# wulibingbinglin/COMET-Pose-Estimation

Measured on AMD Instinct MI355X. Metric: sequences/sec (BxT frames) COMET fwd+bwd, T=16 512^2, higher is better.
Workload: dtype bf16; 1 GPU; train_e2epose2.py fwd+bwd (COMET tracker+DINOv2+head, loss, backward, grad all-reduce, clip 1.0, AdamW) -- BASELINE configs[2]; global_batch=8, seq_len=16, image=512, tracks=512, parallelism=dp1

## Files before the change

### comet-pose-estimation_amd/comet_amd/_lib.py

```python
import ctypes
import os

_HERE = os.path.dirname(os.path.abspath(__file__))
_DEFAULT_LIB = "libcomet_hip_debug.so" if os.environ.get("COMET_DEBUG") == "1" else "libcomet_hip.so"
LIB_PATH = os.environ.get("COMET_HIP_LIB", os.path.join(os.path.dirname(_HERE), _DEFAULT_LIB))

F32 = 0
BF16 = 1
ACT_NONE, ACT_GELU, ACT_RELU, ACT_SIGMOID = 0, 1, 2, 3
SQ_NORM_PARTIALS = 1024

c_i64 = ctypes.c_int64
c_i32 = ctypes.c_int32
c_vp = ctypes.c_void_p


class GemmArgs(ctypes.Structure):
    _fields_ = [
        ("dtype_ab", c_i32), ("dtype_c", c_i32), ("layout_a", c_i32), ("layout_b", c_i32),
        ("m", c_i64), ("n", c_i64), ("k", c_i64), ("batch", c_i64 * 2),
        ("a", c_vp), ("lda", c_i64), ("stride_a", c_i64 * 2),
        ("b", c_vp), ("ldb", c_i64), ("stride_b", c_i64 * 2),
        ("c", c_vp), ("ldc", c_i64), ("stride_c", c_i64 * 2),
        ("bias", c_vp), ("bias_mode", c_i32), ("stride_bias", c_i64 * 2),
# ... 22 lines not shown
        ("bias", c_vp),
        ("y", c_vp), ("ldy", c_i64),
        ("resid", c_vp), ("ldr", c_i64), ("beta", ctypes.c_float),
        ("act", c_i32),
    ]


class AttnArgs(ctypes.Structure):
    _fields_ = [
        ("dtype", c_i32), ("head_dim", c_i32),
        ("batch", c_i64), ("heads", c_i64), ("lq", c_i64), ("lk", c_i64),
        ("q", c_vp), ("sq_b", c_i64), ("sq_h", c_i64), ("sq_l", c_i64),
        ("k", c_vp), ("sk_b", c_i64), ("sk_h", c_i64), ("sk_l", c_i64),
        ("v", c_vp), ("sv_b", c_i64), ("sv_h", c_i64), ("sv_l", c_i64),
        ("o", c_vp), ("so_b", c_i64), ("so_h", c_i64), ("so_l", c_i64),
        ("lse", c_vp), ("scale", ctypes.c_float),
        ("batch_inner", c_i64), ("sq_i", c_i64), ("sk_i", c_i64), ("sv_i", c_i64), ("so_i", c_i64),
    ]


class AttnBwdArgs(ctypes.Structure):
    _fields_ = [
        ("dtype", c_i32), ("head_dim", c_i32),
        ("batch", c_i64), ("heads", c_i64), ("lq", c_i64), ("lk", c_i64),
        ("q", c_vp), ("sq_b", c_i64), ("sq_h", c_i64), ("sq_l", c_i64),
        ("k", c_vp), ("sk_b", c_i64), ("sk_h", c_i64), ("sk_l", c_i64),
        ("v", c_vp), ("sv_b", c_i64), ("sv_h", c_i64), ("sv_l", c_i64),
        ("o", c_vp), ("so_b", c_i64), ("so_h", c_i64), ("so_l", c_i64),
        ("dout", c_vp), ("sd_b", c_i64), ("sd_h", c_i64), ("sd_l", c_i64),
        ("dq", c_vp), ("sdq_b", c_i64), ("sdq_h", c_i64), ("sdq_l", c_i64),
        ("dk", c_vp), ("sdk_b", c_i64), ("sdk_h", c_i64), ("sdk_l", c_i64),
        ("dv", c_vp), ("sdv_b", c_i64), ("sdv_h", c_i64), ("sdv_l", c_i64),
        ("lse", c_vp), ("delta", c_vp), ("scale", ctypes.c_float),
    ]


class RingTensor(ctypes.Structure):
    _fields_ = [("src", c_vp), ("dst", c_vp), ("slot_bytes", c_i64)]


RING_MAX_TENSORS = 4
FUSE_ROW = 20
CARRY_MAX_TRACKS, CARRY_MAX_CANDIDATES, CARRY_MAX_CELLS = 4096, 65536, 8192
LM_ROW = 12
PNP_MAX_ITERS = 16

_F = ctypes.c_float
_INT = ctypes.c_int
SIGNATURES = {
    "comet_count_nonfinite": (_INT, [_INT, c_vp, c_i64, c_vp, c_vp]),
    "comet_debug_flags": (_INT, [_INT]),
    "comet_lds_probe": (_INT, [_INT, _INT, _INT, c_vp, c_vp]),
    "comet_shfl_probe": (_INT, [_INT, _INT, _INT, c_vp, c_vp]),
    "comet_version": (_INT, []),
    "comet_last_error": (ctypes.c_char_p, []),
    "comet_gemm": (_INT, [ctypes.POINTER(GemmArgs), c_vp]),
    "comet_gemm_workspace": (_INT, [ctypes.POINTER(GemmArgs), ctypes.POINTER(c_i64)]),
    "comet_gemm_plan": (_INT, [ctypes.POINTER(GemmArgs), ctypes.POINTER(c_i64), ctypes.POINTER(ctypes.c_int32)]),
    "comet_gemm_rowln_ok": (_INT, [ctypes.POINTER(GemmArgs)]),
    "comet_gemm_rowln_workspace": (_INT, [ctypes.POINTER(GemmArgs), ctypes.POINTER(ctypes.c_int64)]),
    "comet_gemm_rowln": (_INT, [ctypes.POINTER(GemmArgs), ctypes.POINTER(RowLNArgs), c_vp]),
    "comet_gemm_dact_ok": (_INT, [ctypes.POINTER(GemmArgs), _INT, c_vp, c_i64]),
    "comet_gemm_dact": (_INT, [ctypes.POINTER(GemmArgs), _INT, c_vp, c_i64, c_vp, c_vp]),
    "comet_conv2d_nhwc": (_INT, [ctypes.POINTER(ConvArgs), c_vp]),
    "comet_conv_plan": (_INT, [ctypes.POINTER(ConvArgs), ctypes.POINTER(ctypes.c_int32)]),
    "comet_layernorm_fwd": (_INT, [_INT, _INT, c_vp, c_vp, c_vp, c_vp, c_vp, c_vp, c_vp, c_i64, c_i64, c_i64, c_i64,
                                   c_i64, _F, _INT, c_vp]),
    "comet_layernorm_bwd": (_INT, [_INT, _INT, c_vp, c_vp, c_vp, c_vp, c_vp, c_vp, _INT, c_vp, c_vp, c_vp, c_i64, c_i64,
                                   _INT, c_vp]),
    "comet_layernorm_bwd_res": (_INT, [_INT, _INT, c_vp, c_vp, c_vp, c_vp, c_vp, c_vp, c_vp, c_vp, c_vp, c_i64, c_i64,
                                       c_vp]),
    "comet_attention_bwd": (_INT, [ctypes.POINTER(AttnBwdArgs), c_vp]),
    "comet_attention_fwd": (_INT, [ctypes.POINTER(AttnArgs), c_vp]),
    "comet_attn_probs": (_INT, [_INT, c_vp, c_vp, c_vp, c_i64, c_i64, c_i64, c_i64, _F, c_vp]),
    "comet_attn_delta": (_INT, [_INT, c_vp, c_vp, c_vp, c_i64, c_i64, c_i64, c_i64, c_i64, c_i64, c_i64, c_i64, c_i64, c_i64, c_vp]),
    "comet_attn_dsoftmax": (_INT, [_INT, c_vp, c_vp, c_vp, c_vp, c_i64, c_i64, c_i64, _F, c_vp]),
    "comet_cast": (_INT, [_INT, _INT, c_vp, c_vp, c_i64, c_vp]),
    "comet_cast_multi_f32_bf16": (_INT, [c_vp, c_vp, c_vp, _INT, c_vp]),
    "comet_act_bwd": (_INT, [_INT, _INT, _INT, c_vp, c_vp, c_vp, _INT, c_i64, c_vp]),
    "comet_axpby": (_INT, [c_vp, c_vp, _F, _F, c_i64, c_vp]),
    "comet_act_bwd_colsum": (_INT, [_INT, _INT, c_vp, _INT, c_vp, _INT, c_vp, c_vp, c_i64, c_i64, _INT, c_vp]),
    "comet_colsum": (_INT, [_INT, c_vp, c_vp, c_i64, c_i64, c_i64, _INT, c_vp]),
    "comet_sq_norm_multi": (_INT, [c_vp, c_vp, _INT, c_vp, c_vp, c_vp]),
    "comet_adamw_multi": (_INT, [c_vp, c_vp, c_vp, c_vp, c_vp, _INT, _F, _F, _F, _F, _F, _INT, c_vp, _F, c_vp]),
    "comet_im2col_nhwc": (_INT, [_INT, _INT, c_vp, c_vp, c_i64, c_i64, c_i64, c_i64, _INT, _INT, _INT, _INT, c_i64, c_i64, c_i64, c_vp]),
    "comet_instnorm_workspace": (_INT, [c_i64, c_i64, c_i64, ctypes.POINTER(c_i64)]),
    "comet_instnorm_nhwc": (_INT, [_INT, c_vp, c_vp, c_vp, c_i64, c_i64, c_i64, _F, _INT, _INT, c_vp, c_i64, c_vp]),
    "comet_resize_bilinear": (_INT, [_INT, _INT, _INT, c_vp, c_vp, c_i64, c_i64, c_i64, c_i64, c_i64, c_i64, _INT, c_vp]),
    "comet_resize_bilinear_pool_nhwc": (_INT, [_INT, _INT, c_vp, c_vp, c_vp, c_i64, c_i64, c_i64, c_i64, c_i64, c_i64, c_vp]),
    "comet_conv1x1_resize_pool_nhwc": (_INT, [c_vp, c_vp, c_i64, c_i64, c_vp, c_i64, c_i64, c_vp, c_vp, c_vp, c_vp, c_vp,
                                               c_i64, c_i64, c_i64, c_i64, c_i64, c_i64, c_vp]),
    "comet_shallow_front_nhwc": (_INT, [_INT, c_vp, c_vp, c_vp, c_vp, c_vp, c_vp, c_i64, c_i64, c_i64, _F, c_vp]),
    "comet_resize_bilinear_nhwc_into": (_INT, [_INT, _INT, c_vp, c_vp, c_i64, c_i64, c_i64, c_i64, c_i64, c_i64, c_i64,
                                               _INT, c_vp]),
    "comet_act_fwd": (_INT, [_INT, _INT, _INT, c_vp, c_vp, c_i64, c_vp]),
    "comet_binary": (_INT, [_INT, _INT, c_vp, c_vp, c_vp, c_i64, c_vp]),
    "comet_add_rows": (_INT, [_INT, _INT, c_vp, c_vp, c_vp, c_i64, c_i64, c_i64, c_i64, c_i64, c_vp]),
    "comet_rowscale_fwd": (_INT, [_INT, c_vp, c_vp, c_vp, c_i64, c_i64, c_vp]),
    "comet_rowscale_bwd": (_INT, [_INT, c_vp, c_vp, c_vp, c_vp, c_vp, c_i64, c_i64, c_vp]),
    "comet_sincos_table": (_INT, [c_vp, c_vp, c_i64, _INT, c_i64, c_i64, c_vp]),
    "comet_harmonic_fwd": (_INT, [c_vp, c_vp, c_vp, c_vp, c_i64, _INT, _INT, _INT, c_vp]),
    "comet_pose_pair_errors": (_INT, [c_vp, c_vp, c_i64, c_i64, c_vp, c_vp, c_vp]),
    "comet_pose_frame_errors": (_INT, [c_vp, c_i64, c_vp, c_i64, c_i64, c_vp, c_vp, c_vp, c_vp]),
    "comet_harmonic_bwd": (_INT, [c_vp, c_vp, c_vp, c_vp, c_vp, c_vp, c_i64, _INT, _INT, _INT, c_vp]),
# ... 77 lines not shown
```

### comet-pose-estimation_amd/comet_amd/functional.py

```python
import contextlib

import os

import torch

from . import _lib as L
from . import ops


class _State:
    dtype = torch.bfloat16


_state = _State()


def compute_dtype():
    return _state.dtype


@contextlib.contextmanager
def precision(dtype):
    old = _state.dtype
    _state.dtype = dtype
# ... 561 lines not shown
        dw = torch.zeros(C, device=x.device) if ctx.needs_input_grad[1] else None
        db = torch.zeros(C, device=x.device) if ctx.needs_input_grad[2] else None
        dx = ops.layernorm_bwd(x, dpre, mean, rstd, w, dw, db) if (ctx.needs_input_grad[0] or dw is not None or db is not None) else None
        return dx, dw, db, None


def layer_norm_relu(x, w, b, eps=1e-5):
    if _needs_grad(x, w, b):
        return _LayerNormReLU.apply(x, w, b, eps)
    return ops.layernorm(x, w, b, eps=eps, out_dtype=torch.float32, relu=True)


class _RowScale(torch.autograd.Function):

    @staticmethod
    def forward(ctx, x, w):
        ctx.save_for_backward(x, w)
        return ops.rowscale(x, w)

    @staticmethod
    def backward(ctx, dy):
        x, w = ctx.saved_tensors
        dx, dw = ops.rowscale_bwd(x, w, dy, ctx.needs_input_grad[0], ctx.needs_input_grad[1])
        return dx, dw


def rowscale(x, w):
    w = w.reshape(x.shape[:-1])
    if _needs_grad(x, w):
        return _RowScale.apply(x, w)
    return ops.rowscale(x, w)


class _Add(torch.autograd.Function):
    @staticmethod
    def forward(ctx, a, b):
        return ops.add(a, b)

    @staticmethod
    def backward(ctx, g):
        return g, g


def add(a, b):
    if _needs_grad(a, b):
        return _Add.apply(a, b)
    return ops.add(a, b)


class _AddRows(torch.autograd.Function):
    @staticmethod
    def forward(ctx, x, table, period):
        return ops.add_rows(x, table, period, out_dtype=torch.float32)

    @staticmethod
    def backward(ctx, g):
        return g, None, None


def add_rows(x, table, period):
    if _needs_grad(x):
        return _AddRows.apply(x, table, period)
    return ops.add_rows(x, table, period, out_dtype=torch.float32)


class _GAPR(torch.autograd.Function):
# ... 89 lines not shown
```

### comet-pose-estimation_amd/comet_amd/models/camera_predictor10.py

```python
import math

import torch
import torch.nn as nn

from .. import _lib as L
from .. import functional as F
from .. import ops
from .dinov2 import dinov2_vitb14_reg
from .modules import AttnBlock, CrossAttnBlock, Mlp
from .utils import INTRINSICS, PredCameras

_RESNET_MEAN = [0.485, 0.456, 0.406]
_RESNET_STD = [0.229, 0.224, 0.225]


class FeatureFusion(nn.Module):

    def __init__(self, rgb_dim, fmap_dim, fusion_type="adaptive"):
        super().__init__()
        self.fusion_type = fusion_type
        self.fmap_proj = nn.Sequential(nn.Linear(fmap_dim, rgb_dim), nn.LayerNorm(rgb_dim), nn.ReLU())
        self.fusion_layer = nn.Linear(rgb_dim * 2, rgb_dim)
        self.out_norm = nn.LayerNorm(rgb_dim)

# ... 146 lines not shown
        blk, cblk = self.self_att[-1], self.cross_att[-1]
        a = blk.attn
        x = tok.reshape(B * S, P, C)
        xn, xc = F.layer_norm_dual(x, eps=1e-6)
        idx = self._query_rows(B, S, P, x.device)
        qin = F.gather_rows(xc.reshape(B * S * P, C), idx)
        rin = F.gather_rows(xn.reshape(B * S * P, C), idx)
        q, kv = F.linear_pair(qin, xc, a.in_proj_weight, a.in_proj_bias, C)
        o0 = F.attention(q[:B * P].reshape(B, P, C), kv.reshape(B, S, P, 2 * C)[:, 0], blk.heads, C)
        o1 = F.attention(q[B * P:].reshape(B * S, 1, C), kv, blk.heads, C)
        o = torch.cat([o0.reshape(B * P, C), o1.reshape(B * S, C)])
        y = F.linear(o, a.out_proj.weight, a.out_proj.bias, resid=rin, out_dtype=torch.float32)
        yr, yn = F.res_layer_norm(y, eps=1e-6)
        y = blk.mlp(yn, resid=yr)
        f0 = y[:B * P].reshape(B, P, C)
        rows = y[B * P:].reshape(B, S, C)[:, 1:].contiguous()
        r = cblk(rows, f0)
        return torch.cat([f0[:, 0:1], r], dim=1)

    def forward(self, reshaped_image, preliminary_cameras=None, iters=4, batch_size=None, rgb_feat_init=None,
                gt_cameras=None, fmaps=None, pred_trajectories=None, track_confidence=None, debug=False,
                tokens=None):
        if rgb_feat_init is None:
            rgb_feat, B, S, C = self.get_2D_image_features(reshaped_image, batch_size, tokens=tokens)
        else:
            rgb_feat = rgb_feat_init
            B, S, C = rgb_feat.shape
        if pred_trajectories is not None and self.USE_TP and self.TP_RESIDUAL:
            traj = self.traj_encoder(pred_trajectories)
            N = traj.shape[2]
            ca = self.confidence_attention
            w = F.linear(track_confidence.unsqueeze(-1), ca[0].weight, ca[0].bias, act=L.ACT_RELU)
            w = F.linear(w, ca[2].weight, ca[2].bias, act=L.ACT_SIGMOID, out_dtype=torch.float32)
            ctx = F.rowscale(traj, w).reshape(B * S, N, C)
            r = rgb_feat.reshape(B * S, 1, C)
            for blk in self.cross_attn_block:
                r = blk(r, ctx)
            rgb_feat = F.add(rgb_feat, r.reshape(B, S, C))
        if self.USE_TIME:
            rgb_feat = F.add_rows(rgb_feat, self._table("1d", S, C, rgb_feat.device), S)
            with F.precision(torch.float32):
                for blk in self.trunk:
                    rgb_feat = blk(rgb_feat)
        if self.SINGLE_HEAD:
            return self._single_head(rgb_feat, gt_cameras, B, S)
        gt_enc = None
        if gt_cameras is not None:
            gt_enc = ops.pose_encode(gt_cameras.R.float(), gt_cameras.T_uvz.float(), gt_cameras.focal_length.float(),
                                     _ratio(gt_cameras), B, S)
        rot = self.pose_branch(rgb_feat)
        uv = F.linear(rgb_feat, self.fc_translation2d.weight, self.fc_translation2d.bias, out_dtype=torch.float32)
        dd = F.linear(rgb_feat, self.fc_depth.weight, self.fc_depth.bias, out_dtype=torch.float32)
        enc, losses = F.gapr(rot, uv, dd, gt_enc, B, S, self._cfg_get("weight_trans", 1), self._cfg_get("weight_rot", 2))
        pred_cameras = None
        if gt_cameras is not None:
            intr = INTRINSICS[_dataset(self.cfg)]
            R, T = ops.pose_decode(enc, gt_cameras.R.float(), gt_cameras.T_uvz.float(), _ratio(gt_cameras), intr, B, S)
            pred_cameras = PredCameras(R=R, T=T, focal_length=torch.zeros(B * S, 0, device=R.device))
        out = {"pred_pose_enc": enc, "gt_pose_enc": gt_enc, "pred_cameras": pred_cameras}
        if gt_enc is not None:
            out.update(loss=losses[0], loss_trans=losses[1], loss_rot=losses[2])
        else:
            out.update(loss=0, loss_trans=0, loss_rot=0)
        return out

    def _single_head(self, rgb_feat, gt_cameras, B, S):
        pred = self.pose_branch(rgb_feat)
        gt8 = None
        if gt_cameras is not None:
            gt8 = ops.pose_encode3(gt_cameras.R.float(), gt_cameras.T.float(), B, S)
# ... 24 lines not shown
```

### comet-pose-estimation_amd/comet_amd/models/modules.py

```python

import torch
import torch.nn as nn

from .. import _lib as L
from .. import functional as F
from .. import ops


class Mlp(nn.Module):
    def __init__(self, in_features, hidden_features=None, out_features=None, act_layer=nn.GELU,
                 norm_layer=None, bias=True, drop=0.0, use_conv=False):
        super().__init__()
        out_features = out_features or in_features
        hidden_features = hidden_features or in_features
        self.fc1 = nn.Linear(in_features, hidden_features, bias=bias)
        self.act = act_layer()
        self.drop1 = nn.Dropout(drop)
        self.fc2 = nn.Linear(hidden_features, out_features, bias=bias)
        self.drop2 = nn.Dropout(drop)

    def forward(self, x, resid=None, out_dtype=torch.float32):
        return F.mlp(x, self.fc1.weight, self.fc1.bias, self.fc2.weight, self.fc2.bias, resid=resid, out_dtype=out_dtype)


# ... 61 lines not shown


@torch.no_grad()
def attn_block_pre(blk, pre, out):
    x32, x16 = pre
    a = blk.attn
    qkv = F.linear(x16, a.in_proj_weight, a.in_proj_bias)
    o = F.attention(qkv, None, blk.heads, x32.shape[-1])
    return _mlp_pre(blk, a, o, x32, out)


@torch.no_grad()
def cross_block_pre(blk, pre, ctx16, out):
    x32, x16 = pre
    C = x32.shape[-1]
    a = blk.cross_attn
    W, b = a.in_proj_weight, a.in_proj_bias
    q = F.linear(x16, W[:C], b[:C])
    kv = F.linear(ctx16, W[C:], b[C:])
    o = F.attention(q, kv, blk.heads, C)
    return _mlp_pre(blk, a, o, x32, out)


class CrossAttnBlock(nn.Module):
    def __init__(self, hidden_size, context_dim, num_heads=1, mlp_ratio=4.0, **kw):
        super().__init__()
        self.norm1 = nn.LayerNorm(hidden_size, elementwise_affine=False, eps=1e-6)
        self.norm_context = nn.LayerNorm(hidden_size)
        self.norm2 = nn.LayerNorm(hidden_size, elementwise_affine=False, eps=1e-6)
        self.cross_attn = _mha_holder(hidden_size, num_heads)
        self.mlp = Mlp(in_features=hidden_size, hidden_features=int(hidden_size * mlp_ratio), drop=0)
        self.heads = num_heads

    def forward(self, x, context, mask=None):
        C = x.shape[-1]
        a = self.cross_attn
        x, xc = F.layer_norm_dual(x, eps=1e-6)
        ctx = F.layer_norm(context, self.norm_context.weight, self.norm_context.bias, eps=1e-5,
                           out_dtype=F.compute_dtype())
        q, kv = F.linear_pair(xc, ctx, a.in_proj_weight, a.in_proj_bias, C)
        o = F.attention(q, kv, self.heads, C)
        x = F.linear(o, a.out_proj.weight, a.out_proj.bias, resid=x, out_dtype=torch.float32)
        xr, xn = F.res_layer_norm(x, eps=1e-6)
        return self.mlp(xn, resid=xr)


def conv2d_nhwc(x, conv, stride, pad, out_dtype=None):
    w = conv.weight
    cout, cin, kh, kw = w.shape
    cx = x.shape[-1]
    wm = F.wcast_conv(w, cin_pad=cx)
    if kh == 1 and kw == 1 and stride == 1 and pad == 0:
        n, h, wd, c = x.shape
        y = F.linear(x.reshape(-1, c), wm, conv.bias, out_dtype=out_dtype)
        return y.reshape(n, h, wd, cout)
    xc = x if x.dtype == wm.dtype else ops.cast(x, wm.dtype)
    if wm.dtype == torch.bfloat16 and cx % 8 == 0:
        return ops.conv2d_nhwc(xc, wm, kh, kw, stride, pad, bias=conv.bias, out_dtype=out_dtype or wm.dtype)
    cols, oh, ow = ops.im2col_nhwc(xc, kh, kw, stride, pad, out_dtype=wm.dtype, ldc=wm.shape[1])
    y = F.linear(cols, wm, conv.bias, out_dtype=out_dtype)
    return y.reshape(x.shape[0], oh, ow, cout)


class ResidualBlock(nn.Module):
    def __init__(self, in_planes, planes, norm_fn="group", stride=1, kernel_size=3):
        super().__init__()
        if norm_fn != "instance":
            raise NotImplementedError("the COMET path only uses norm_fn='instance'")
        self.conv1 = nn.Conv2d(in_planes, planes, kernel_size=kernel_size, padding=1, stride=stride)
        self.conv2 = nn.Conv2d(planes, planes, kernel_size=kernel_size, padding=1)
        self.relu = nn.ReLU(inplace=True)
        self.norm1 = nn.InstanceNorm2d(planes)
# ... 17 lines not shown
```

### comet-pose-estimation_amd/comet_amd/ops.py

```python
import ctypes
from typing import NamedTuple

import torch

from . import _lib as L
from .profiler import PROF

_DT = {torch.float32: L.F32, torch.bfloat16: L.BF16}


def dt(t):
    try:
        return _DT[t.dtype]
    except KeyError:
        raise L.CometHipError(f"unsupported dtype {t.dtype}") from None


def stream():
    return ctypes.c_void_p(torch.cuda.current_stream().cuda_stream)


def _p(t):
    return None if t is None else t.data_ptr()

# ... 913 lines not shown
    r = _rows2d(x)
    xc = x
    if r is None:
        xc = x.contiguous()
        r = _rows2d(xc)
    rows, ldx = r
    y = out if out is not None else torch.empty(x.shape, device=x.device, dtype=out_dtype or x.dtype)
    ry = _rows2d(y)
    _chk(L.load().comet_add_rows(dt(xc), dt(y), _p(xc), _p(table), _p(y), rows, C, period, ldx, ry[1], stream()),
         "add_rows")
    return y


def rowscale(x, w):
    xc = x.contiguous()
    C = x.shape[-1]
    y = torch.empty_like(xc)
    _chk(L.load().comet_rowscale_fwd(dt(xc), _p(xc), _p(w), _p(y), xc.numel() // C, C, stream()), "rowscale")
    return y


def rowscale_bwd(x, w, dy, need_dx=True, need_dw=True):
    xc = x.contiguous()
    C = x.shape[-1]
    rows = xc.numel() // C
    dyc = dy.contiguous().float() if dy.dtype != torch.float32 else dy.contiguous()
    dx = torch.empty(x.shape, device=x.device, dtype=torch.float32) if need_dx else None
    dw = torch.empty(w.shape, device=x.device, dtype=torch.float32) if need_dw else None
    _chk(L.load().comet_rowscale_bwd(dt(xc), _p(xc), _p(w), _p(dyc), _p(dx), _p(dw), rows, C, stream()),
         "rowscale_bwd")
    return dx, dw


def sincos_table(pos, dim, out=None, col0=0):
    pos = pos.contiguous().float()
    m = pos.numel()
    if out is None:
        out = torch.empty(m, dim, device=pos.device, dtype=torch.float32)
    _chk(L.load().comet_sincos_table(_p(pos), _p(out), m, dim, out.stride(0), col0, stream()), "sincos")
    return out


def sincos_2d(embed_dim, gh, gw, device):
    xs = torch.arange(gw, device=device, dtype=torch.float32).repeat(gh)
    ys = torch.arange(gh, device=device, dtype=torch.float32).repeat_interleave(gw)
    out = torch.empty(gh * gw, embed_dim, device=device, dtype=torch.float32)
    sincos_table(xs, embed_dim // 2, out=out, col0=0)
    sincos_table(ys, embed_dim // 2, out=out, col0=embed_dim // 2)
    return out


def _ratio_args(ratio):
    if torch.is_tensor(ratio):
        if ratio.is_cuda:
            r = ratio.reshape(-1)[:1].to(torch.float64).contiguous()
            return 0.0, r, _p(r)
        return float(ratio.reshape(-1)[0]), None, None
    return float(ratio), None, None


def pose_encode(R, T_uvz, focal, ratio, B, S):
    enc = torch.empty(B * S, 8, device=R.device, dtype=torch.float32)
    rh, keep, rd = _ratio_args(ratio)
    _chk(L.load().comet_pose_encode(_p(R.contiguous()), _p(T_uvz.contiguous()), _p(focal.contiguous()),
                                    rh, rd, _p(enc), B, S, stream()), "pose_encode")
    return enc
# ... 184 lines not shown
        if not PROF.enabled or _TIMED_DEPTH[0] > 0:
            return fn(*args, **kwargs)
        if PROF.detail:
            f = sys._getframe(1)
            while f is not None and f.f_code.co_filename.endswith("ops.py"):
                f = f.f_back
            sites = []
            while f is not None and len(sites) < 2:
                sites.append(f"{os.path.basename(f.f_code.co_filename)}:{f.f_lineno}")
                f = f.f_back
            site = "<".join(sites) or "?"
            shapes = ",".join("x".join(map(str, a.shape)) + str(a.dtype)[6:] for a in args if isinstance(a, torch.Tensor))
            name = f"{fn.__name__} [{shapes}] @{site}"
        else:
            name = "comet_" + fn.__name__
        e0 = PROF.start()
        _TIMED_DEPTH[0] += 1
        try:
            out = fn(*args, **kwargs)
        finally:
            _TIMED_DEPTH[0] -= 1
        nb = _gather_bytes(fn.__name__, args, out)
        if nb is None:
            seen = set()
            nb = _tensor_bytes(args, seen) + _tensor_bytes(kwargs.values(), seen)
            nb += _tensor_bytes(out if isinstance(out, (list, tuple)) else (out,), seen)
        PROF.stop(e0, name, 0.0, float(nb))
        return out
    return wrap


for _name in ("layernorm", "layernorm_bwd", "layernorm_bwd_res", "cast", "cast_multi_f32_bf16", "act_bwd", "colsum",
              "act_bwd_colsum", "instnorm_nhwc", "resize_bilinear", "resize_bilinear_into", "resize_bilinear_pool", "conv1x1_resize_pool", "im2col_nhwc", "act_fwd",
              "binary", "add_rows", "rowscale", "rowscale_bwd", "sample_bilinear", "corr_sample", "tracker_tokens",
              "coords_update", "avgpool2_nhwc", "patch_gather", "refine_combine", "track_score", "dino_prep",
              "pose_encode", "pose_decode", "pose_encode3", "pose_decode3", "images_nhwc", "harmonic_fwd",
              "harmonic_bwd", "sincos_table"):
    globals()[_name] = _timed(globals()[_name])
```

### include/comet_hip.h

```cpp
#ifndef COMET_HIP_H_
#define COMET_HIP_H_

#include <stdint.h>
#include <stddef.h>

#ifdef __cplusplus
extern "C" {
#endif

#define COMET_F32 0
#define COMET_BF16 1

#define COMET_OK 0
#define COMET_EINVAL -1
#define COMET_ELAUNCH -2

#define COMET_ACT_NONE 0
#define COMET_ACT_GELU 1
#define COMET_ACT_RELU 2
#define COMET_ACT_SIGMOID 3

int comet_version(void);
const char* comet_last_error(void);

// ... 31 lines not shown
int comet_gemm_rowln(const comet_gemm_args* args, const comet_rowln_args* ln, void* stream);

int comet_gemm_dact_ok(const comet_gemm_args* args, int32_t act, const void* pre, int64_t ldpre);
int comet_gemm_dact(const comet_gemm_args* args, int32_t act, const void* pre, int64_t ldpre, float* dbias,
                    void* stream);


typedef struct comet_conv_args {
  int32_t dtype;
  int32_t dtype_y;
  const void* x; int64_t n, h, w, c;
  const void* weight; int64_t cout, ldw;
  int32_t kh, kw, stride, pad;
  const float* bias;
  void* y; int64_t ldy;
  const void* resid; int64_t ldr; float beta;
  int32_t act;
} comet_conv_args;

int comet_conv2d_nhwc(const comet_conv_args* args, void* stream);
int comet_conv_plan(const comet_conv_args* args, int32_t* plan);

int comet_layernorm_fwd(int dtype_x, int dtype_y, const void* x, const float* weight,
                        const float* bias, void* y, void* y2, float* mean, float* rstd,
                        int64_t rows, int64_t cols, int64_t ldx, int64_t ldy, int64_t ldy2,
                        float eps, int relu, void* stream);
int comet_layernorm_bwd(int dtype_x, int dtype_dy, const void* x, const void* dy, const void* dy2,
                        const float* mean, const float* rstd, const float* weight,
                        int dtype_dx, void* dx, float* dweight, float* dbias, int64_t rows, int64_t cols,
                        int dx_accumulate, void* stream);
int comet_layernorm_bwd_res(int dtype_x, int dtype_dy, const void* x, const void* dy, const float* dres,
                            const float* mean, const float* rstd, const float* weight, float* dx,
                            float* dweight, float* dbias, int64_t rows, int64_t cols, void* stream);

typedef struct comet_attn_args {
  int32_t dtype;
  int32_t head_dim;
  int64_t batch, heads, lq, lk;
  const void* q; int64_t sq_b, sq_h, sq_l;
  const void* k; int64_t sk_b, sk_h, sk_l;
  const void* v; int64_t sv_b, sv_h, sv_l;
  void* o; int64_t so_b, so_h, so_l;
  float* lse;
  float scale;
  int64_t batch_inner;
  int64_t sq_i, sk_i, sv_i, so_i;
} comet_attn_args;

int comet_attention_fwd(const comet_attn_args* args, void* stream);

typedef struct comet_attn_bwd_args {
  int32_t dtype;
  int32_t head_dim;
  int64_t batch, heads, lq, lk;
  const void* q; int64_t sq_b, sq_h, sq_l;
  const void* k; int64_t sk_b, sk_h, sk_l;
  const void* v; int64_t sv_b, sv_h, sv_l;
  const void* o; int64_t so_b, so_h, so_l;
  const void* dout; int64_t sd_b, sd_h, sd_l;
  void* dq; int64_t sdq_b, sdq_h, sdq_l;
  void* dk; int64_t sdk_b, sdk_h, sdk_l;
  void* dv; int64_t sdv_b, sdv_h, sdv_l;
  const float* lse;
  float* delta;
  float scale;
} comet_attn_bwd_args;
// ... 198 lines not shown
```

Baseline: 70.07 sequences/s.

## Fuse rowscale with multiple context layernorms for cross-attention blocks

Adds a HIP kernel that applies the per-row confidence scale and a single shared layernorm, then writes one bf16 output per cross-attention block's affine params. A matching backward kernel accumulates dx, dw, dgamma and dbeta in one pass. This replaces a rowscale followed by a separate layernorm in each block, so the f32 context tensor is read once instead of several times and fewer kernels launch. It relies on all blocks sharing the same eps, and it accumulates dgamma/dbeta with atomics.

```diff
diff --git a/comet-pose-estimation_amd/comet_amd/_lib.py b/comet-pose-estimation_amd/comet_amd/_lib.py
--- a/comet-pose-estimation_amd/comet_amd/_lib.py
+++ b/comet-pose-estimation_amd/comet_amd/_lib.py
@@ -78,6 +78,19 @@
         ("dk", c_vp), ("sdk_b", c_i64), ("sdk_h", c_i64), ("sdk_l", c_i64),
         ("dv", c_vp), ("sdv_b", c_i64), ("sdv_h", c_i64), ("sdv_l", c_i64),
         ("lse", c_vp), ("delta", c_vp), ("scale", ctypes.c_float),
+    ]
+
+
+RSLN_MAX = 4
+
+
+class RowScaleLNArgs(ctypes.Structure):
+    _fields_ = [
+        ("x", c_vp), ("w", c_vp), ("rows", c_i64), ("cols", c_i64), ("eps", ctypes.c_float), ("n", c_i32),
+        ("gamma", c_vp * RSLN_MAX), ("beta", c_vp * RSLN_MAX), ("y", c_vp * RSLN_MAX),
+        ("mean", c_vp), ("rstd", c_vp),
+        ("dy", c_vp * RSLN_MAX), ("dx", c_vp), ("dw", c_vp),
+        ("dgamma", c_vp * RSLN_MAX), ("dbeta", c_vp * RSLN_MAX),
     ]
 
 
@@ -116,6 +129,9 @@
                                    _INT, c_vp]),
     "comet_layernorm_bwd_res": (_INT, [_INT, _INT, c_vp, c_vp, c_vp, c_vp, c_vp, c_vp, c_vp, c_vp, c_vp, c_i64, c_i64,
                                        c_vp]),
+    "comet_rowscale_ln_multi_fwd": (_INT, [ctypes.POINTER(RowScaleLNArgs), c_vp]),
+    "comet_rowscale_ln_multi_bwd": (_INT, [ctypes.POINTER(RowScaleLNArgs), c_vp]),
+    "comet_rowscale_ln_multi_ok": (_INT, [c_i64, _INT, c_vp]),
     "comet_attention_bwd": (_INT, [ctypes.POINTER(AttnBwdArgs), c_vp]),
     "comet_attention_fwd": (_INT, [ctypes.POINTER(AttnArgs), c_vp]),
     "comet_attn_probs": (_INT, [_INT, c_vp, c_vp, c_vp, c_i64, c_i64, c_i64, c_i64, _F, c_vp]),
diff --git a/comet-pose-estimation_amd/comet_amd/functional.py b/comet-pose-estimation_amd/comet_amd/functional.py
--- a/comet-pose-estimation_amd/comet_amd/functional.py
+++ b/comet-pose-estimation_amd/comet_amd/functional.py
@@ -617,6 +617,53 @@
     return ops.rowscale(x, w)
 
 
+class _RowScaleLNMulti(torch.autograd.Function):
+
+    @staticmethod
+    def forward(ctx, x, w, eps, *affine):
+        n = len(affine) // 2
+        gammas, betas = affine[:n], affine[n:]
+        ys, mean, rstd = ops.rowscale_ln_multi(x, w, gammas, betas, eps)
+        ctx.save_for_backward(x, w, mean, rstd, *gammas)
+        ctx.set_materialize_grads(False)
+        ctx.n, ctx.eps = n, eps
+        return tuple(ys)
+
+    @staticmethod
+    def backward(ctx, *dys):
+        x, w, mean, rstd, *gammas = ctx.saved_tensors
+        n = ctx.n
+        if all(d is None for d in dys):
+            return (None,) * (3 + 2 * n)
+        need = ctx.needs_input_grad
+        affine = [need[3 + i] or need[3 + n + i] for i in range(n)]
+        dx, dw, dgs, dbs = ops.rowscale_ln_multi_bwd(x, w, mean, rstd, gammas, dys, need[0], need[1], affine, ctx.eps)
+        dgs = [g if need[3 + i] else None for i, g in enumerate(dgs)]
+        dbs = [b if need[3 + n + i] else None for i, b in enumerate(dbs)]
+        return (dx, dw, None, *dgs, *dbs)
+
+
+def rowscale_ln_multi(x, w, norms, eps=1e-5):
+    w = w.reshape(x.shape[:-1])
+    norms = [(m.weight, m.bias) if isinstance(m, torch.nn.Module) else m for m in norms]
+    gammas = [g for g, _ in norms]
+    betas = [b for _, b in norms]
+    x = x.contiguous()
+    w = w.contiguous()
+    if _needs_grad(x, w, *gammas, *betas):
+        return list(_RowScaleLNMulti.apply(x, w, eps, *gammas, *betas))
+    return ops.rowscale_ln_multi(x, w, gammas, betas, eps)[0]
+
+
+def tp_ctx_fused(x, norms):
+    if os.environ.get("COMET_TP_CTX_FUSE", "1") == "0" or compute_dtype() != torch.bfloat16:
+        return False
+    if not 1 <= len(norms) <= 4 or any(m.eps != norms[0].eps for m in norms):
+        return False
+    params = [p for m in norms for p in (m.weight, m.bias)]
+    return ops.rowscale_ln_multi_ok(x, len(norms), params)
+
+
 class _Add(torch.autograd.Function):
     @staticmethod
     def forward(ctx, a, b):
diff --git a/comet-pose-estimation_amd/comet_amd/models/camera_predictor10.py b/comet-pose-estimation_amd/comet_amd/models/camera_predictor10.py
--- a/comet-pose-estimation_amd/comet_amd/models/camera_predictor10.py
+++ b/comet-pose-estimation_amd/comet_amd/models/camera_predictor10.py
@@ -202,10 +202,16 @@
             ca = self.confidence_attention
             w = F.linear(track_confidence.unsqueeze(-1), ca[0].weight, ca[0].bias, act=L.ACT_RELU)
             w = F.linear(w, ca[2].weight, ca[2].bias, act=L.ACT_SIGMOID, out_dtype=torch.float32)
-            ctx = F.rowscale(traj, w).reshape(B * S, N, C)
             r = rgb_feat.reshape(B * S, 1, C)
-            for blk in self.cross_attn_block:
-                r = blk(r, ctx)
+            norms = [blk.norm_context for blk in self.cross_attn_block]
+            if F.tp_ctx_fused(traj, norms):
+                ctxs = F.rowscale_ln_multi(traj, w, norms, norms[0].eps)
+                for blk, c16 in zip(self.cross_attn_block, ctxs):
+                    r = blk(r, None, ctx16=c16.reshape(B * S, N, C))
+            else:
+                ctx = F.rowscale(traj, w).reshape(B * S, N, C)
+                for blk in self.cross_attn_block:
+                    r = blk(r, ctx)
             rgb_feat = F.add(rgb_feat, r.reshape(B, S, C))
         if self.USE_TIME:
             rgb_feat = F.add_rows(rgb_feat, self._table("1d", S, C, rgb_feat.device), S)
diff --git a/comet-pose-estimation_amd/comet_amd/models/modules.py b/comet-pose-estimation_amd/comet_amd/models/modules.py
--- a/comet-pose-estimation_amd/comet_amd/models/modules.py
+++ b/comet-pose-estimation_amd/comet_amd/models/modules.py
@@ -117,12 +117,14 @@
         self.mlp = Mlp(in_features=hidden_size, hidden_features=int(hidden_size * mlp_ratio), drop=0)
         self.heads = num_heads
 
-    def forward(self, x, context, mask=None):
+    def forward(self, x, context, mask=None, ctx16=None):
         C = x.shape[-1]
         a = self.cross_attn
         x, xc = F.layer_norm_dual(x, eps=1e-6)
-        ctx = F.layer_norm(context, self.norm_context.weight, self.norm_context.bias, eps=1e-5,
-                           out_dtype=F.compute_dtype())
+        ctx = ctx16
+        if ctx is None:
+            ctx = F.layer_norm(context, self.norm_context.weight, self.norm_context.bias, eps=1e-5,
+                               out_dtype=F.compute_dtype())
         q, kv = F.linear_pair(xc, ctx, a.in_proj_weight, a.in_proj_bias, C)
         o = F.attention(q, kv, self.heads, C)
         x = F.linear(o, a.out_proj.weight, a.out_proj.bias, resid=x, out_dtype=torch.float32)
diff --git a/comet-pose-estimation_amd/comet_amd/ops.py b/comet-pose-estimation_amd/comet_amd/ops.py
--- a/comet-pose-estimation_amd/comet_amd/ops.py
+++ b/comet-pose-estimation_amd/comet_amd/ops.py
@@ -969,6 +969,68 @@
     return dx, dw
 
 
+def rowscale_ln_multi_ok(x, n, params=()):
+    if x.dtype != torch.float32 or not x.is_cuda or not x.is_contiguous():
+        return False
+    for p in params:
+        if p is None or p.dtype != torch.float32 or not p.is_contiguous() or p.data_ptr() % 16 or p.numel() != x.shape[-1]:
+            return False
+    return bool(L.load().comet_rowscale_ln_multi_ok(x.shape[-1], int(n), _p(x)))
+
+
+def _rsln_args(x, w, gammas, eps):
+    C = x.shape[-1]
+    a = L.RowScaleLNArgs()
+    a.x, a.w, a.rows, a.cols, a.eps, a.n = _p(x), _p(w), x.numel() // C, C, float(eps), len(gammas)
+    for i, g in enumerate(gammas):
+        a.gamma[i] = _p(g)
+    return a
+
+
+def rowscale_ln_multi(x, w, gammas, betas, eps=1e-5):
+    _req_cuda(x)
+    n = len(gammas)
+    if not 1 <= n <= L.RSLN_MAX or len(betas) != n:
+        raise L.CometHipError(f"rowscale_ln_multi: 1..{L.RSLN_MAX} (gamma, beta) pairs, got {n}")
+    if x.dtype != torch.float32 or not x.is_contiguous() or not w.is_contiguous() or w.numel() * x.shape[-1] != x.numel():
+        raise L.CometHipError("rowscale_ln_multi: x must be contiguous f32 [..., C] and w contiguous f32 [...]")
+    rows = w.numel()
+    a = _rsln_args(x, w, gammas, eps)
+    ys = [torch.empty(x.shape, device=x.device, dtype=torch.bfloat16) for _ in range(n)]
+    mean = torch.empty(rows, device=x.device, dtype=torch.float32)
+    rstd = torch.empty(rows, device=x.device, dtype=torch.float32)
+    for i in range(n):
+        a.beta[i], a.y[i] = _p(betas[i]), _p(ys[i])
+    a.mean, a.rstd = _p(mean), _p(rstd)
+    _chk(L.load().comet_rowscale_ln_multi_fwd(ctypes.byref(a), stream()), "rowscale_ln_multi")
+    return ys, mean, rstd
+
+
+def rowscale_ln_multi_bwd(x, w, mean, rstd, gammas, dys, need_dx=True, need_dw=True, need_affine=None, eps=1e-5):
+    n = len(gammas)
+    a = _rsln_args(x, w, gammas, eps)
+    a.mean, a.rstd = _p(mean), _p(rstd)
+    C = x.shape[-1]
+    dx = torch.empty(x.shape, device=x.device, dtype=torch.float32) if need_dx else None
+    dw = torch.empty(w.shape, device=x.device, dtype=torch.float32) if need_dw else None
+    a.dx, a.dw = _p(dx), _p(dw)
+    keep, dgs, dbs = [], [None] * n, [None] * n
+    for i, dy in enumerate(dys):
+        if dy is None:
+            continue
+        if dy.dtype != torch.bfloat16:
+            raise L.CometHipError("rowscale_ln_multi_bwd: dy must be bf16")
+        dyc = dy.contiguous()
+        keep.append(dyc)
+        a.dy[i] = _p(dyc)
+        if need_affine is None or need_affine[i]:
+            dgs[i] = torch.zeros(C, device=x.device, dtype=torch.float32)
+            dbs[i] = torch.zeros(C, device=x.device, dtype=torch.float32)
+            a.dgamma[i], a.dbeta[i] = _p(dgs[i]), _p(dbs[i])
+    _chk(L.load().comet_rowscale_ln_multi_bwd(ctypes.byref(a), stream()), "rowscale_ln_multi_bwd")
+    return dx, dw, dgs, dbs
+
+
 def sincos_table(pos, dim, out=None, col0=0):
     pos = pos.contiguous().float()
     m = pos.numel()
@@ -1219,7 +1281,7 @@
 
 for _name in ("layernorm", "layernorm_bwd", "layernorm_bwd_res", "cast", "cast_multi_f32_bf16", "act_bwd", "colsum",
               "act_bwd_colsum", "instnorm_nhwc", "resize_bilinear", "resize_bilinear_into", "resize_bilinear_pool", "conv1x1_resize_pool", "im2col_nhwc", "act_fwd",
-              "binary", "add_rows", "rowscale", "rowscale_bwd", "sample_bilinear", "corr_sample", "tracker_tokens",
+              "binary", "add_rows", "rowscale", "rowscale_bwd", "rowscale_ln_multi", "rowscale_ln_multi_bwd", "sample_bilinear", "corr_sample", "tracker_tokens",
               "coords_update", "avgpool2_nhwc", "patch_gather", "refine_combine", "track_score", "dino_prep",
               "pose_encode", "pose_decode", "pose_encode3", "pose_decode3", "images_nhwc", "harmonic_fwd",
               "harmonic_bwd", "sincos_table"):
diff --git a/comet-pose-estimation_amd/csrc/tp_ctx.hip b/comet-pose-estimation_amd/csrc/tp_ctx.hip
--- /dev/null
+++ b/comet-pose-estimation_amd/csrc/tp_ctx.hip
@@ -0,0 +1,342 @@
+#include <cstdlib>
+
+#include "common.hpp"
+
+#pragma clang fp contract(off)
+
+namespace comet {
+namespace {
+
+constexpr int RS_CH = 4;
+
+template <int NK, int N>
+__global__ void __launch_bounds__(256)
+rsln_fwd_kernel(comet_rowscale_ln_args a) {
+  constexpr int CH = RS_CH;
+  const int lane = threadIdx.x & 63;
+  const int cols = (int)a.cols;
+  const int64_t rows = a.rows;
+  const int64_t nw = (int64_t)gridDim.x * 4;
+  int64_t row = (int64_t)blockIdx.x * 4 + (threadIdx.x >> 6);
+  if (row >= rows) return;
+  float gv[N][NK][CH], bv[N][NK][CH];
+#pragma unroll
+  for (int i = 0; i < N; ++i)
+#pragma unroll
+    for (int k = 0; k < NK; ++k) {
+      const int c0 = (lane + 64 * k) * CH;
+      if (c0 < cols) {
+        load4(a.gamma[i] + c0, gv[i][k]);
+        load4(a.beta[i] + c0, bv[i][k]);
+      } else {
+#pragma unroll
+        for (int e = 0; e < CH; ++e) { gv[i][k][e] = 1.f; bv[i][k][e] = 0.f; }
+      }
+    }
+  float v[NK][CH], nx[NK][CH];
+  float wr, nwr = 0.f;
+  auto load_row = [&](int64_t r, float (&dst)[NK][CH], float& wd) {
+    wd = a.w[r];
+#pragma unroll
+    for (int k = 0; k < NK; ++k) {
+      const int c0 = (lane + 64 * k) * CH;
+      if (c0 < cols) {
+        load4(a.x + r * cols + c0, dst[k]);
+      } else {
+#pragma unroll
+        for (int e = 0; e < CH; ++e) dst[k][e] = 0.f;
+      }
+    }
+  };
+  load_row(row, v, wr);
+  for (; row < rows; row += nw) {
+    const int64_t nrow = row + nw;
+    if (nrow < rows) load_row(nrow, nx, nwr);
+    float s = 0.f;
+#pragma unroll
+    for (int k = 0; k < NK; ++k) {
+      const int c0 = (lane + 64 * k) * CH;
+#pragma unroll
+      for (int e = 0; e < CH; ++e) {
+        if (c0 < cols) v[k][e] = v[k][e] * wr;
+        s += v[k][e];
+      }
+    }
+    const float mean = wave_sum(s) / cols;
+    float q = 0.f;
+#pragma unroll
+    for (int k = 0; k < NK; ++k) {
+      const int c0 = (lane + 64 * k) * CH;
+      if (c0 >= cols) continue;
+      float d[CH];
+#pragma unroll
+      for (int e = 0; e < CH; ++e) d[e] = v[k][e] - mean;
+      if (k == 0) {
+        q = __builtin_fmaf(d[0], d[0], d[1] * d[1]);
+        q = __builtin_fmaf(d[2], d[2], q);
+        q = __builtin_fmaf(d[3], d[3], q);
+      } else {
+#pragma unroll
+        for (int e = 0; e < CH; ++e) q = __builtin_fmaf(d[e], d[e], q);
+      }
+    }
+    const float var = wave_sum(q) / cols;
+    const float rstd = rsqrtf(var + a.eps);
+#pragma unroll
+    for (int k = 0; k < NK; ++k) {
+      const int c0 = (lane + 64 * k) * CH;
+      if (c0 >= cols) continue;
+      float h[CH];
+#pragma unroll
+      for (int e = 0; e < CH; ++e) h[e] = (v[k][e] - mean) * rstd;
+#pragma unroll
+      for (int i = 0; i < N; ++i) {
+        float o[CH];
+#pragma unroll
+        for (int e = 0; e < CH; ++e) o[e] = h[e] * gv[i][k][e] + bv[i][k][e];
+        store4((__bf16*)a.y[i] + row * cols + c0, o);
+      }
+    }
+    if (lane == 0) {
+      a.mean[row] = mean;
+      a.rstd[row] = rstd;
+    }
+    wr = nwr;
+#pragma unroll
+    for (int k = 0; k < NK; ++k)
+#pragma unroll
+      for (int e = 0; e < CH; ++e) v[k][e] = nx[k][e];
+  }
+}
+
+__device__ __forceinline__ void unpack4(const uint2& u, float (&v)[4]) {
+  v[0] = bf16_lo(u.x); v[1] = bf16_hi(u.x); v[2] = bf16_lo(u.y); v[3] = bf16_hi(u.y);
+}
+
+__device__ __forceinline__ void wave_lds_sync() {
+  __builtin_amdgcn_fence(__ATOMIC_RELEASE, "wavefront");
+  __builtin_amdgcn_wave_barrier();
+  __builtin_amdgcn_fence(__ATOMIC_ACQUIRE, "wavefront");
+}
+
+template <int NK, int N>
+__global__ void __launch_bounds__(256)
+rsln_bwd_kernel(comet_rowscale_ln_args a, int rpw) {
+  constexpr int CH = RS_CH;
+  __shared__ float red[4][1024];
+  const int lane = threadIdx.x & 63, wid = threadIdx.x >> 6;
+  const int cols = (int)a.cols;
+  const int64_t rows = a.rows;
+  float gw[N][NK][CH], gb[N][NK][CH], gam[N][NK][CH];
+#pragma unroll
+  for (int i = 0; i < N; ++i)
+#pragma unroll
+    for (int k = 0; k < NK; ++k) {
+      const int c0 = (lane + 64 * k) * CH;
+#pragma unroll
+      for (int e = 0; e < CH; ++e) { gw[i][k][e] = 0.f; gb[i][k][e] = 0.f; gam[i][k][e] = 1.f; }
+      if (c0 < cols) load4(a.gamma[i] + c0, gam[i][k]);
+    }
+  const int64_t rbase = ((int64_t)blockIdx.x * 4 + wid) * rpw;
+  for (int rr = 0; rr < rpw; ++rr) {
+    const int64_t row = rbase + rr;
+    if (row >= rows) break;
+    const float mu = a.mean[row], rs = a.rstd[row], wr = a.w[row];
+    float xv[NK][CH], xh[NK][CH];
+    uint2 draw[N][NK];
+#pragma unroll
+    for (int k = 0; k < NK; ++k) {
+      const int c0 = (lane + 64 * k) * CH;
+      if (c0 < cols) {
+        load4(a.x + row * cols + c0, xv[k]);
+#pragma unroll
+        for (int i = 0; i < N; ++i)
+          draw[i][k] = a.dy[i] ? *reinterpret_cast<const uint2*>((const __bf16*)a.dy[i] + row * cols + c0) : uint2{0, 0};
+      } else {
+#pragma unroll
+        for (int e = 0; e < CH; ++e) xv[k][e] = 0.f;
+#pragma unroll
+        for (int i = 0; i < N; ++i) draw[i][k] = uint2{0, 0};
+      }
+    }
+#pragma unroll
+    for (int k = 0; k < NK; ++k) {
+      const int c0 = (lane + 64 * k) * CH;
+#pragma unroll
+      for (int e = 0; e < CH; ++e) xh[k][e] = c0 < cols ? (xv[k][e] * wr - mu) * rs : 0.f;
+    }
+    float s1[N], s2[N];
+#pragma unroll
+    for (int i = 0; i < N; ++i) {
+      s1[i] = 0.f; s2[i] = 0.f;
+      if (!a.dy[i]) continue;
+#pragma unroll
+      for (int k = 0; k < NK; ++k) {
+        const int c0 = (lane + 64 * k) * CH;
+        if (c0 >= cols) continue;
+        float d[CH];
+        unpack4(draw[i][k], d);
+#pragma unroll
+        for (int e = 0; e < CH; ++e) {
+          gw[i][k][e] = __builtin_fmaf(d[e], xh[k][e], gw[i][k][e]);
+          gb[i][k][e] = d[e] + gb[i][k][e];
+          const float g = d[e] * gam[i][k][e];
+          s1[i] = __builtin_fmaf(d[e], gam[i][k][e], s1[i]);
+          s2[i] = __builtin_fmaf(xh[k][e], g, s2[i]);
+        }
+      }
+    }
+#pragma unroll
+    for (int i = 0; i < N; ++i) {
+      s1[i] = wave_sum(s1[i]) / cols;
+      s2[i] = wave_sum(s2[i]) / cols;
+    }
+    float acc[NK][CH];
+    bool have = false;
+#pragma unroll
+    for (int i = N - 1; i >= 0; --i) {
+      if (!a.dy[i]) continue;
+#pragma unroll
+      for (int k = 0; k < NK; ++k) {
+        float d[CH];
+        unpack4(draw[i][k], d);
+#pragma unroll
+        for (int e = 0; e < CH; ++e) {
+          const float g = d[e] * gam[i][k][e];
+          const float o = rs * __builtin_fmaf(-s2[i], xh[k][e], g - s1[i]);
+          acc[k][e] = have ? acc[k][e] + o : o;
+        }
+      }
+      have = true;
+    }
+    float* lrow = red[wid];
+#pragma unroll
+    for (int k = 0; k < NK; ++k) {
+      const int c0 = (lane + 64 * k) * CH;
+      if (c0 >= cols) continue;
+      float o[CH], p[CH];
+#pragma unroll
+      for (int e = 0; e < CH; ++e) { o[e] = acc[k][e] * wr; p[e] = acc[k][e] * xv[k][e]; }
+      if (a.dx) store4(a.dx + row * cols + c0, o);
+      if (a.dw) store4(lrow + c0, p);
+    }
+    if (a.dw) {
+      wave_lds_sync();
+      float s = 0.f;
+      for (int c = lane; c < cols; c += 64) s += lrow[c];
+      s = wave_sum(s);
+      if (lane == 0) a.dw[row] = s;
+      wave_lds_sync();
+    }
+  }
+#pragma unroll
+  for (int i = 0; i < N; ++i) {
+    if (!a.dy[i]) continue;
+#pragma unroll
+    for (int t = 0; t < 2; ++t) {
+      float* dst = t == 0 ? a.dgamma[i] : a.dbeta[i];
+      if (!dst) continue;
+      __syncthreads();
+#pragma unroll
+      for (int k = 0; k < NK; ++k) {
+        const int c0 = (lane + 64 * k) * CH;
+        if (c0 < cols) store4(red[wid] + c0, t == 0 ? gw[i][k] : gb[i][k]);
+      }
+      __syncthreads();
+      for (int c = threadIdx.x; c < cols; c += 256) atomicAdd(dst + c, red[0][c] + red[1][c] + red[2][c] + red[3][c]);
+    }
+  }
+}
+
+bool rsln_a32(const void* p) { return ((uintptr_t)p % 32) == 0; }
+bool rsln_a16(const void* p) { return ((uintptr_t)p % 16) == 0; }
+
+int rsln_env(const char* name, int lo, int hi) {
+  if (const char* e = getenv(name)) {
+    const int v = atoi(e);
+    if (v >= lo && v <= hi) return v;
+  }
+  return 0;
+}
+
+bool rsln_shape_ok(int64_t cols, int n) {
+  return cols > 0 && cols <= 1024 && cols % 8 == 0 && n >= 1 && n <= COMET_RSLN_MAX;
+}
+
+}
+}
+
+using namespace comet;
+
+extern "C" int comet_rowscale_ln_multi_ok(int64_t cols, int n, const void* ptr) {
+  return rsln_shape_ok(cols, n) && rsln_a32(ptr) ? 1 : 0;
+}
+
+#define RSLN_DISPATCH(KERNEL, ...)                                                        \
+  do {                                                                                    \
+    const int nk = (int)cdiv(a.cols, 64 * RS_CH);                                         \
+    switch ((nk - 1) * 4 + (a.n - 1)) {                                                   \
+      case 0: KERNEL(1, 1, __VA_ARGS__); break;  case 1: KERNEL(1, 2, __VA_ARGS__); break;  \
+      case 2: KERNEL(1, 3, __VA_ARGS__); break;  case 3: KERNEL(1, 4, __VA_ARGS__); break;  \
+      case 4: KERNEL(2, 1, __VA_ARGS__); break;  case 5: KERNEL(2, 2, __VA_ARGS__); break;  \
+      case 6: KERNEL(2, 3, __VA_ARGS__); break;  case 7: KERNEL(2, 4, __VA_ARGS__); break;  \
+      case 8: KERNEL(3, 1, __VA_ARGS__); break;  case 9: KERNEL(3, 2, __VA_ARGS__); break;  \
+      case 10: KERNEL(3, 3, __VA_ARGS__); break; case 11: KERNEL(3, 4, __VA_ARGS__); break; \
+      case 12: KERNEL(4, 1, __VA_ARGS__); break; case 13: KERNEL(4, 2, __VA_ARGS__); break; \
+      case 14: KERNEL(4, 3, __VA_ARGS__); break; default: KERNEL(4, 4, __VA_ARGS__); break; \
+    }                                                                                     \
+  } while (0)
+
+extern "C" int comet_rowscale_ln_multi_fwd(const comet_rowscale_ln_args* args, void* stream) {
+  COMET_CHECK_ARG(args, "comet_rowscale_ln_multi_fwd: null args");
+  const comet_rowscale_ln_args a = *args;
+  COMET_CHECK_ARG(rsln_shape_ok(a.cols, a.n),
+                  "comet_rowscale_ln_multi_fwd: needs cols % 8 == 0, cols in [8,1024] and 1 <= n <= 4");
+  COMET_CHECK_ARG(a.rows >= 0 && a.rows < (1ll << 40), "comet_rowscale_ln_multi_fwd: bad rows");
+  COMET_CHECK_ARG(a.x && a.w && a.mean && a.rstd, "comet_rowscale_ln_multi_fwd: null pointer");
+  COMET_CHECK_ARG(rsln_a32(a.x), "comet_rowscale_ln_multi_fwd: x must be 32-B aligned");
+  for (int i = 0; i < a.n; ++i) {
+    COMET_CHECK_ARG(a.gamma[i] && a.beta[i] && a.y[i], "comet_rowscale_ln_multi_fwd: null gamma / beta / y");
+    COMET_CHECK_ARG(rsln_a32(a.y[i]) && rsln_a16(a.gamma[i]) && rsln_a16(a.beta[i]),
+                    "comet_rowscale_ln_multi_fwd: y must be 32-B, gamma / beta 16-B aligned");
+  }
+  if (a.rows == 0) return COMET_OK;
+  int64_t wgs = 256 * 3;
+  if (const int v = rsln_env("COMET_TP_CTX_WGS", 1, 65536)) wgs = v;
+  const int64_t iters = cdiv(a.rows, wgs * 4);
+  const dim3 grid((unsigned)cdiv(cdiv(a.rows, iters), 4));
+  hipStream_t s = as_stream(stream);
+#define RSLN_F(NK, N, unused) hipLaunchKernelGGL((rsln_fwd_kernel<NK, N>), grid, dim3(256), 0, s, a)
+  RSLN_DISPATCH(RSLN_F, 0);
+#undef RSLN_F
+  COMET_CHECK_LAUNCH("comet_rowscale_ln_multi_fwd");
+  return COMET_OK;
+}
+
+extern "C" int comet_rowscale_ln_multi_bwd(const comet_rowscale_ln_args* args, void* stream) {
+  COMET_CHECK_ARG(args, "comet_rowscale_ln_multi_bwd: null args");
+  const comet_rowscale_ln_args a = *args;
+  COMET_CHECK_ARG(rsln_shape_ok(a.cols, a.n),
+                  "comet_rowscale_ln_multi_bwd: needs cols % 8 == 0, cols in [8,1024] and 1 <= n <= 4");
+  COMET_CHECK_ARG(a.rows >= 0 && a.rows < (1ll << 40), "comet_rowscale_ln_multi_bwd: bad rows");
+  COMET_CHECK_ARG(a.x && a.w && a.mean && a.rstd, "comet_rowscale_ln_multi_bwd: null pointer");
+  COMET_CHECK_ARG(rsln_a32(a.x) && rsln_a32(a.dx), "comet_rowscale_ln_multi_bwd: x / dx must be 32-B aligned");
+  bool any = false, affine = false;
+  for (int i = 0; i < a.n; ++i) {
+    COMET_CHECK_ARG(a.gamma[i] && rsln_a16(a.gamma[i]), "comet_rowscale_ln_multi_bwd: gamma must be non-null, 16-B aligned");
+    COMET_CHECK_ARG(rsln_a32(a.dy[i]), "comet_rowscale_ln_multi_bwd: dy must be 32-B aligned");
+    any = any || a.dy[i];
+    affine = affine || (a.dy[i] && (a.dgamma[i] || a.dbeta[i]));
+  }
+  COMET_CHECK_ARG(any, "comet_rowscale_ln_multi_bwd: every dy is null");
+  if (a.rows == 0) return COMET_OK;
+  int rpw = affine ? 16 : 2;
+  if (const int v = rsln_env("COMET_LNB_RPW", 1, 64)) rpw = v;
+  const dim3 grid((unsigned)cdiv(a.rows, 4 * rpw));
+  hipStream_t s = as_stream(stream);
+#define RSLN_B(NK, N, unused) hipLaunchKernelGGL((rsln_bwd_kernel<NK, N>), grid, dim3(256), 0, s, a, rpw)
+  RSLN_DISPATCH(RSLN_B, 0);
+#undef RSLN_B
+  COMET_CHECK_LAUNCH("comet_rowscale_ln_multi_bwd");
+  return COMET_OK;
+}
diff --git a/include/comet_hip.h b/include/comet_hip.h
--- a/include/comet_hip.h
+++ b/include/comet_hip.h
@@ -87,6 +87,28 @@
 int comet_layernorm_bwd_res(int dtype_x, int dtype_dy, const void* x, const void* dy, const float* dres,
                             const float* mean, const float* rstd, const float* weight, float* dx,
                             float* dweight, float* dbias, int64_t rows, int64_t cols, void* stream);
+
+#define COMET_RSLN_MAX 4
+typedef struct comet_rowscale_ln_args {
+  const float* x;
+  const float* w;
+  int64_t rows, cols;
+  float eps;
+  int32_t n;
+  const float* gamma[COMET_RSLN_MAX];
+  const float* beta[COMET_RSLN_MAX];
+  void* y[COMET_RSLN_MAX];
+  float* mean;
+  float* rstd;
+  const void* dy[COMET_RSLN_MAX];
+  float* dx;
+  float* dw;
+  float* dgamma[COMET_RSLN_MAX];
+  float* dbeta[COMET_RSLN_MAX];
+} comet_rowscale_ln_args;
+int comet_rowscale_ln_multi_fwd(const comet_rowscale_ln_args* args, void* stream);
+int comet_rowscale_ln_multi_bwd(const comet_rowscale_ln_args* args, void* stream);
+int comet_rowscale_ln_multi_ok(int64_t cols, int n, const void* ptr);
 
 typedef struct comet_attn_args {
   int32_t dtype;
```

New measurement: 70.65 sequences/s (median of 6 runs). No clear change (+0.8%).
